# zhu-edward/DGSQP

Measured on NVIDIA B200. Metric: converged_game_solves_per_sec, higher is better.
Workload: dtype f64

## Files before the change

dgsqp_b200/csrc/cta.cuh:

```cuda
#pragma once
#include <math.h>
#include <stdint.h>

enum { PH_LIN_FULL = 0, PH_ADJ_FULL, PH_HESS, PH_PD_TRIDIAG, PH_PD_EIG, PH_CHOL, PH_TRINV, PH_GI, PH_LSQR,
       PH_LIN_GRAD, PH_ADJ_GRAD, PH_MERIT, PH_OTHER,
       PH_PD_SYM, PH_PD_EIGVAL, PH_PD_INVIT, PH_PD_BACK, PH_GI_SLACK, PH_GI_DZ, PH_GI_STEP, PH_GI_ADD, PH_GI_DROP, PH_QP_X0, PH_QP_WARM,
       PH_WS_D, PH_WS_QR, PH_WS_APPLY, PH_WS_MULT,
       DG_NPHASE };

#ifdef DG_HOSTSIM
#define DG_RSQRT(x) (1.0 / sqrt(x))
#define DG_ATOMIC_MIN(p, v) do { if ((v) < *(p)) *(p) = (v); } while (0)
#define DG_DEV static inline
#define DG_HD static inline
#define DG_DEVN static
#define DG_CONST static const
#define DG_RESTRICT
struct Cta {
  inline int tid() const { return 0; }
  inline int nt() const { return 1; }
  inline int lane() const { return 0; }
  inline int warp() const { return 0; }
  inline int nwarps() const { return 1; }
  static constexpr int wsz = 1;
  double* red = nullptr;
  inline void sync() {}
  inline double sum(double v) { return v; }
  inline double max(double v) { return v; }
  inline void max3(double& a, double& b, double& d) {}
  inline double min(double v) { return v; }
  inline int imin(int v) { return v; }
  inline int isum(int v) { return v; }
  inline void argmin(double v, int idx, double& ov, int& oi) { ov = v; oi = idx; }
  inline double warp_sum(double v) { return v; }
  template <int N> inline void warp_sum_n(double (&)[N]) {}
  inline void warp_argmin(double&, int&) {}
  inline void syncwarp() {}
  inline void sum2(double& a, double& b) {}
  inline void sum3(double& a, double& b, double& d) {}
  inline void sum4(double& a, double& b, double& d, double& e) {}
  inline int bcast0(int v) { return v; }
  inline void lap(int) {}
  inline void lapf(int) {}
  inline void lap2(int, int) {}
};
#else
#define DG_RSQRT(x) rsqrt(x)
#define DG_ATOMIC_MIN(p, v) atomicMin((p), (v))
#define DG_DEV __device__ __forceinline__
#define DG_HD __host__ __device__ __forceinline__
#define DG_DEVN __device__ __noinline__
#define DG_CONST __device__ const
#ifdef DG_NO_RESTRICT
#define DG_RESTRICT
#else
#define DG_RESTRICT __restrict__
#endif
__shared__ __align__(16) double dg_s_red[320];
__shared__ long long dg_s_ph[DG_NPHASE + 1];

struct Cta {
  __device__ __forceinline__ int tid() const { return (int)threadIdx.x; }
  __device__ __forceinline__ int nt() const { return (int)blockDim.x; }
  __device__ __forceinline__ int lane() const { return (int)(threadIdx.x & 31u); }
  __device__ __forceinline__ int warp() const { return (int)(threadIdx.x >> 5); }
  __device__ __forceinline__ int nwarps() const { return (int)((blockDim.x + 31u) >> 5); }
  static constexpr int wsz = 32;
  __device__ __forceinline__ void lap(int id) {
    if (tid() == 0) { long long t = clock64(); dg_s_ph[id] += t - dg_s_ph[DG_NPHASE]; dg_s_ph[DG_NPHASE] = t; }
  }
#ifdef DG_FINE_PHASES
  __device__ __forceinline__ void lapf(int id) { lap(id); }
  __device__ __forceinline__ void lap2(int, int fine) { lap(fine); }
#else
  __device__ __forceinline__ void lapf(int) {}
  __device__ __forceinline__ void lap2(int coarse, int) { lap(coarse); }
#endif
  __device__ __forceinline__ void sync() { __syncthreads(); }
  __device__ __forceinline__ double warp_sum(double v) {
#pragma unroll
    for (int o = 16; o > 0; o >>= 1) v += __shfl_xor_sync(0xffffffffu, v, o);
    return v;
  }
  template <int N>
  __device__ __forceinline__ void warp_sum_n(double (&v)[N]) {
#pragma unroll
    for (int o = 16; o > 0; o >>= 1) {
#pragma unroll
      for (int t = 0; t < N; ++t) v[t] += __shfl_xor_sync(0xffffffffu, v[t], o);
    }
  }
  __device__ __forceinline__ void warp_argmin(double& v, int& idx) {
#pragma unroll
    for (int o = 16; o > 0; o >>= 1) {
      const double v2 = __shfl_xor_sync(0xffffffffu, v, o);
      const int i2 = __shfl_xor_sync(0xffffffffu, idx, o);
      if (v2 < v || (v2 == v && i2 < idx)) { v = v2; idx = i2; }
    }
  }
  int flip = 0;
  __device__ __forceinline__ double* next_buf() { flip ^= 1; return dg_s_red + flip * 160; }
  __device__ __forceinline__ void syncwarp() { __syncwarp(); }
  __device__ __forceinline__ double tree16(const double* b) const {
    if (nwarps() == 8) {
      const double2 p0 = reinterpret_cast<const double2*>(b)[0], p1 = reinterpret_cast<const double2*>(b)[1];
      const double2 p2 = reinterpret_cast<const double2*>(b)[2], p3 = reinterpret_cast<const double2*>(b)[3];
      return ((p0.x + p0.y) + (p1.x + p1.y)) + ((p2.x + p2.y) + (p3.x + p3.y));
    }
    double t[16];
#pragma unroll
    for (int w = 0; w < 16; ++w) t[w] = w < nwarps() ? b[w] : 0.0;
#pragma unroll
    for (int s = 8; s > 0; s >>= 1)
#pragma unroll
      for (int w = 0; w < s; ++w) t[w] += t[w + s];
    return t[0];
  }
  __device__ __forceinline__ double sum(double v) {
    v = warp_sum(v);
    double* b = next_buf();
    if (lane() == 0) b[warp()] = v;
    __syncthreads();
    return tree16(b);
  }
  __device__ __forceinline__ void sum2(double& a0, double& a1) {
    a0 = warp_sum(a0); a1 = warp_sum(a1);
    double* b = next_buf();
    if (lane() == 0) { b[warp()] = a0; b[32 + warp()] = a1; }
    __syncthreads();
    a0 = tree16(b); a1 = tree16(b + 32);
  }
  __device__ __forceinline__ void sum3(double& a0, double& a1, double& a2) {
    a0 = warp_sum(a0); a1 = warp_sum(a1); a2 = warp_sum(a2);
    double* b = next_buf();
    if (lane() == 0) { b[warp()] = a0; b[32 + warp()] = a1; b[64 + warp()] = a2; }
    __syncthreads();
    a0 = tree16(b); a1 = tree16(b + 32); a2 = tree16(b + 64);
  }
  __device__ __forceinline__ void sum4(double& a0, double& a1, double& a2, double& a3) {
    a0 = warp_sum(a0); a1 = warp_sum(a1); a2 = warp_sum(a2); a3 = warp_sum(a3);
    double* b = next_buf();
    if (lane() == 0) { b[warp()] = a0; b[32 + warp()] = a1; b[64 + warp()] = a2; b[96 + warp()] = a3; }
    __syncthreads();
    a0 = tree16(b); a1 = tree16(b + 32); a2 = tree16(b + 64); a3 = tree16(b + 96);
  }
  __device__ __forceinline__ double max(double v) {
#pragma unroll
    for (int o = 16; o > 0; o >>= 1) v = fmax(v, __shfl_xor_sync(0xffffffffu, v, o));
    double* b = next_buf();
    if (lane() == 0) b[warp()] = v;
    __syncthreads();
    double r = b[0];
    for (int w = 1; w < nwarps(); ++w) r = fmax(r, b[w]);
    return r;
  }
  __device__ __forceinline__ void max3(double& a0, double& a1, double& a2) {
#pragma unroll
    for (int o = 16; o > 0; o >>= 1) {
      a0 = fmax(a0, __shfl_xor_sync(0xffffffffu, a0, o));
      a1 = fmax(a1, __shfl_xor_sync(0xffffffffu, a1, o));
      a2 = fmax(a2, __shfl_xor_sync(0xffffffffu, a2, o));
    }
    double* b = next_buf();
    if (lane() == 0) { b[warp()] = a0; b[32 + warp()] = a1; b[64 + warp()] = a2; }
    __syncthreads();
    double r0 = b[0], r1 = b[32], r2 = b[64];
    for (int w = 1; w < nwarps(); ++w) { r0 = fmax(r0, b[w]); r1 = fmax(r1, b[32 + w]); r2 = fmax(r2, b[64 + w]); }
    a0 = r0; a1 = r1; a2 = r2;
  }
  __device__ __forceinline__ double min(double v) { return -max(-v); }
  __device__ __forceinline__ int bcast0(int v) {
    int* b = (int*)next_buf();
    if (tid() == 0) b[0] = v;
    __syncthreads();
    return b[0];
  }
  __device__ __forceinline__ int imin(int v) {
#pragma unroll
    for (int o = 16; o > 0; o >>= 1) { int t = __shfl_xor_sync(0xffffffffu, v, o); v = t < v ? t : v; }
    int* b = (int*)next_buf();
    if (lane() == 0) b[warp()] = v;
    __syncthreads();
    int r = b[0];
    for (int w = 1; w < nwarps(); ++w) { int t = b[w]; r = t < r ? t : r; }
    return r;
  }
  __device__ __forceinline__ int isum(int v) {
#pragma unroll
    for (int o = 16; o > 0; o >>= 1) v += __shfl_xor_sync(0xffffffffu, v, o);
    int* b = (int*)next_buf();
    if (lane() == 0) b[warp()] = v;
    __syncthreads();
    int r = 0;
    for (int w = 0; w < nwarps(); ++w) r += b[w];
    return r;
  }
  __device__ __forceinline__ void argmin(double v, int idx, double& ov, int& oi) {
#pragma unroll
    for (int o = 16; o > 0; o >>= 1) {
      double v2 = __shfl_xor_sync(0xffffffffu, v, o);
      int i2 = __shfl_xor_sync(0xffffffffu, idx, o);
      if (v2 < v || (v2 == v && i2 < idx)) { v = v2; idx = i2; }
    }
    double* b = next_buf();
    if (lane() == 0) { b[warp()] = v; ((int*)(b + 32))[warp()] = idx; }
    __syncthreads();
    ov = b[0]; oi = ((int*)(b + 32))[0];
    for (int w = 1; w < nwarps(); ++w) {
      double v2 = b[w]; int i2 = ((int*)(b + 32))[w];
      if (v2 < ov || (v2 == ov && i2 < oi)) { ov = v2; oi = i2; }
    }
  }
};
#endif

#ifdef DG_HOSTSIM
#define DG_ASSUME_SHARED(p) do { } while (0)
#else
#define DG_ASSUME_SHARED(p) do { if (SM) __builtin_assume(__isShared((const void*)(p))); } while (0)
#endif

#ifdef DG_HOSTSIM
#include <chrono>
static inline double dg_now_ns() { return (double)std::chrono::duration_cast<std::chrono::nanoseconds>(std::chrono::steady_clock::now().time_since_epoch()).count(); }
#else
__device__ __forceinline__ double dg_now_ns() { unsigned long long t; asm volatile("mov.u64 %0, %%globaltimer;" : "=l"(t)); return (double)t; }
#endif

#define DG_FOR(i, n) for (int i = c.tid(); i < (n); i += c.nt())
#define DG_FOR_OFF(i, n, off) for (int i = (c.tid() + c.nt() - ((off) % c.nt())) % c.nt(); i < (n); i += c.nt())

struct Split2 { int i0, istep, g, G; };
DG_DEV Split2 split2(const Cta& c, int len) {
  int cw = (len + Cta::wsz - 1) / Cta::wsz * Cta::wsz;
  if (cw > c.nt()) cw = c.nt();
  if (cw < 1) cw = 1;
  Split2 s;
  s.G = c.nt() / cw; s.g = c.tid() / cw; s.i0 = c.tid() - s.g * cw; s.istep = cw;
  if (s.g >= s.G) s.i0 = len;
  return s;
}
```

dgsqp_b200/csrc/game_kkt.cuh:

```cuda
#pragma once

template <bool SM>
DG_DEVN void game_constraints(Cta& c, const GameDesc& G, const Dims& D_, const double* u, const double* up,
                              const double* x, double* g, const int* DG_RESTRICT rowtab) {
  const Dims D = D_;
  DG_ASSUME_SHARED(x); DG_ASSUME_SHARED(g); DG_ASSUME_SHARED(up);
  DG_FOR(r, D.m) {
    int k, kind, a, b;
    unpack_row(rowtab[r], k, kind, a, b);
    double val;
    if (kind == K_COLL) {
      double dx = x[k * D.nq + a * DG_NQA] - x[k * D.nq + b * DG_NQA];
      double dy = x[k * D.nq + a * DG_NQA + 1] - x[k * D.nq + b * DG_NQA + 1];
      double rr = G.obs_r[a] + G.obs_r[b];
      val = rr * rr - (dx * dx + dy * dy);
    } else if (kind == K_GAME) val = game_row_value(G, D, u, up, x, k, a, b);
    else if (kind == K_INUB) val = u[uidx(D, a, k, b)] - G.u_ub[b];
    else if (kind == K_INLB) val = G.u_lb[b] - u[uidx(D, a, k, b)];
    else if (kind == K_STUB) val = x[k * D.nq + a * DG_NQA + b] - game_state_ub(G);
    else val = game_state_lb(G) - x[k * D.nq + a * DG_NQA + b];
    g[r] = val;
  }
}

template <bool SM>
DG_DEVN void game_sens(Cta& c, const Dims& D_, const EvalBuf& E_) {
  const EvalBuf E = E_; DG_SH_EVAL(E); const Dims D = D_;
  const int twoN = D.twoN;
  DG_FOR(t, D.M * twoN) {
    int a = t / twoN, j = t - a * twoN, kj = j >> 1, cc = j & 1;
    double s[DG_NQA];
    const double* AB = E.AB + (kj * D.M + a) * DG_AB_SZ;
    for (int i = 0; i < DG_NQA; ++i) s[i] = AB[i * DG_AB_LD + DG_NQA + cc];
    for (int k = kj + 1; k <= D.N; ++k) {
      if (k > kj + 1) {
        const double* Ak = E.AB + ((k - 1) * D.M + a) * DG_AB_SZ;
        double ts[DG_NQA];
        for (int i = 0; i < DG_NQA; ++i) {
          double acc = 0.0;
          for (int jj = 0; jj < DG_NQA; ++jj) acc += Ak[i * DG_AB_LD + jj] * s[jj];
          ts[i] = acc;
        }
        for (int i = 0; i < DG_NQA; ++i) s[i] = ts[i];
      }
      double* Sk = E.S + sens_off(D, a, k, 0) + j;
      Sk[0] = s[0]; Sk[2 * k] = s[1]; Sk[4 * k] = s[DG_BOUND_STATE];
    }
  }
}

template <bool SM>
DG_DEV double sens_dot(const Dims& D, const EvalBuf& E, int a, int k, int row, const double* va) {
  const double* DG_RESTRICT Sk = E.S + sens_off(D, a, k, row);
  double a0 = 0.0, a1 = 0.0;
  for (int j = 0; j < 2 * k; j += 2) { a0 += Sk[j] * va[j]; a1 += Sk[j + 1] * va[j + 1]; }
  return a0 + a1;
}

template <bool SM>
DG_DEVN void game_G_times(Cta& c, const Dims& D_, const EvalBuf& E_, const double* v, double* y) {
  const EvalBuf E = E_; DG_SH_EVAL(E); const Dims D = D_;
  c.sync();
  DG_FOR(t, D.M * D.N * 3) {
    int a = t / (D.N * 3), rem = t - a * D.N * 3, k1 = rem / 3, row = rem - k1 * 3;
    E.tmpS[t] = sens_dot<SM>(D, E, a, k1 + 1, row, v + a * D.twoN);
  }
  c.sync();
  DG_FOR(r, D.m) {
    int k, kind, a, b;
    unpack_row(E.rowtab[r], k, kind, a, b);
    double val;
    if (kind == K_COLL) {
      double dx = E.x[k * D.nq + a * DG_NQA] - E.x[k * D.nq + b * DG_NQA];
      double dy = E.x[k * D.nq + a * DG_NQA + 1] - E.x[k * D.nq + b * DG_NQA + 1];
      const double* ta = E.tmpS + (a * D.N + (k - 1)) * 3;
      const double* tb = E.tmpS + (b * D.N + (k - 1)) * 3;
      val = -2.0 * (dx * (ta[0] - tb[0]) + dy * (ta[1] - tb[1]));
    } else if (kind == K_GAME) val = game_row_Gv(D, E, v, k, a, b);
    else if (kind == K_INUB) val = v[uidx(D, a, k, b)];
    else if (kind == K_INLB) val = -v[uidx(D, a, k, b)];
    else if (kind == K_STUB) val = E.tmpS[(a * D.N + (k - 1)) * 3 + 2];
    else val = -E.tmpS[(a * D.N + (k - 1)) * 3 + 2];
    y[r] = val;
  }
  c.sync();
}

template <bool SM>
DG_DEV void game_state_coefs(Cta& c, const Dims& D, const EvalBuf& E, const double* w, double* cf) {
  DG_FOR(t, D.M * D.N) {
    int a = t / D.N, k = t - a * D.N + 1;
    double cx = 0.0, cy = 0.0;
    for (int p = 0; p < D.P; ++p) {
      int i, j;
      pair_ij(D.M, p, i, j);
      if (i != a && j != a) continue;
      double dx = E.x[k * D.nq + i * DG_NQA] - E.x[k * D.nq + j * DG_NQA];
      double dy = E.x[k * D.nq + i * DG_NQA + 1] - E.x[k * D.nq + j * DG_NQA + 1];
      double wl = w[row_coll(D, k, p)] * (i == a ? -2.0 : 2.0);
      cx += wl * dx; cy += wl * dy;
    }
    game_row_coefs(D, E, w, k, a, cx, cy);
    cf[t * 3] = cx; cf[t * 3 + 1] = cy;
    cf[t * 3 + 2] = w[row_stub(D, k, a)] - w[row_stlb(D, k, a)];
  }
}

DG_DEV double game_GT_direct(const Dims& D, const double* w, int a, int k, int cc) {
  return game_row_GT_direct(D, w, a, k, cc, row_inub(D, k, a, cc), row_inlb(D, k, a, cc));
}

template <bool SM>
DG_DEVN void game_GT_times(Cta& c, const Dims& D_, const EvalBuf& E_, const double* w, double* y) {
  const EvalBuf E = E_; DG_SH_EVAL(E); const Dims D = D_;
  c.sync();
  game_state_coefs<SM>(c, D, E, w, E.cf);
  c.sync();
  DG_FOR(t, D.n) {
    int a = t / D.twoN, j = t - a * D.twoN, kj = j >> 1, cc = j & 1;
    double acc = game_GT_direct(D, w, a, kj, cc);
    for (int k = kj + 1; k <= D.N; ++k) {
      const double* Sk = E.S + sens_off(D, a, k, 0) + j;
      const double* cf = E.cf + (a * D.N + (k - 1)) * 3;
      acc += cf[0] * Sk[0] + cf[1] * Sk[2 * k] + cf[2] * Sk[4 * k];
    }
    y[t] = acc;
  }
  c.sync();
}

DG_DEV double game_G_entry(const Dims& D, const EvalBuf& E, const RowCoef& rc, int k, int kind, int a, int b, int t) {
  int ta = t / D.twoN, j = t - ta * D.twoN, kj = j >> 1, cc = j & 1;
  double val = 0.0;
  if (kind == K_COLL) {
    if ((ta == a || ta == b) && kj < k) {
      double dx = E.x[k * D.nq + a * DG_NQA] - E.x[k * D.nq + b * DG_NQA];
      double dy = E.x[k * D.nq + a * DG_NQA + 1] - E.x[k * D.nq + b * DG_NQA + 1];
      const double* Sk = E.S + sens_off(D, ta, k, 0) + j;
      double sg = ta == a ? -2.0 : 2.0;
      val = sg * (dx * Sk[0] + dy * Sk[2 * k]);
    }
  } else if (kind == K_GAME) game_row_G(D, E, rc, k, a, b, ta, j, kj, cc, val);
  else if (kind == K_INUB) { if (ta == a && kj == k && cc == b) val = 1.0; }
  else if (kind == K_INLB) { if (ta == a && kj == k && cc == b) val = -1.0; }
  else {
    if (ta == a && kj < k) {
      double sv = E.S[sens_off(D, ta, k, 2) + j];
      val = kind == K_STUB ? sv : -sv;
    }
  }
  return val;
}

DG_DEV bool game_G_sparse(const Dims& D, int r, int& t1, int& t2) {
  int k, kind, a, b;
  decode_row(D, r, k, kind, a, b);
  t1 = t2 = -1;
  if (kind == K_INUB) { t1 = uidx(D, a, k, b) << 1; return true; }
  if (kind == K_INLB) { t1 = (uidx(D, a, k, b) << 1) | 1; return true; }
  if (kind == K_GAME) return game_row_sparse(D, k, a, b, t1, t2);
  return false;
}

template <bool SM>
DG_DEVN void game_G_row(Cta& c, const Dims& D_, const EvalBuf& E_, int r, double* out) {
  const EvalBuf E = E_; DG_SH_EVAL(E); const Dims D = D_;
  int k, kind, a, b;
  decode_row(D, r, k, kind, a, b);
  RowCoef rc;
  game_row_prep(D, E, k, kind, a, b, rc);
  DG_FOR(t, D.n) out[t] = game_G_entry(D, E, rc, k, kind, a, b, t);
  c.sync();
}

template <bool SM>
DG_DEVN void game_G_cols(Cta& c, const Dims& D_, const EvalBuf& E_, const int* ids, int cnt, double* out, int ldo) {
  const EvalBuf E = E_; DG_SH_EVAL(E); const Dims D = D_;
  for (int col = c.warp(); col < cnt; col += c.nwarps()) {
    int k, kind, a, b;
    decode_row(D, ids[col], k, kind, a, b);
    RowCoef rc;
    game_row_prep(D, E, k, kind, a, b, rc);
    for (int t = c.lane(); t < D.n; t += c.wsz) out[t * ldo + col] = game_G_entry(D, E, rc, k, kind, a, b, t);
  }
}

DG_DEV double con_lx(const GameDesc& G, const Dims& D, const double* x, const double* l, int k, int idx) {
  int a = idx / DG_NQA, comp = idx - a * DG_NQA;
  if (comp == DG_BOUND_STATE) return l[row_stub(D, k, a)] - l[row_stlb(D, k, a)];
  if (comp > 1) return 0.0;
  double v = 0.0;
  for (int p = 0; p < D.P; ++p) {
    int i, j;
    pair_ij(D.M, p, i, j);
    if (i != a && j != a) continue;
    double dd = x[k * D.nq + i * DG_NQA + comp] - x[k * D.nq + j * DG_NQA + comp];
    v += l[row_coll(D, k, p)] * (i == a ? -2.0 : 2.0) * dd;
  }
  game_row_lx(G, D, x, l, k, a, comp, v);
  return v;
}

DG_DEV double con_lxx(const Dims& D, const double* l, int k, int i1, int i2) {
  int a1 = i1 / DG_NQA, c1 = i1 - a1 * DG_NQA, a2 = i2 / DG_NQA, c2 = i2 - a2 * DG_NQA;
  if (c1 > 1 || c1 != c2) return 0.0;
  double v = 0.0;
  for (int p = 0; p < D.P; ++p) {
    int i, j;
    pair_ij(D.M, p, i, j);
    double lp = l[row_coll(D, k, p)];
    if (a1 == a2) { if (a1 == i || a1 == j) v += -2.0 * lp; }
    else if ((a1 == i && a2 == j) || (a1 == j && a2 == i)) v += 2.0 * lp;
  }
  return v;
}

template <bool SM>
DG_DEVN void game_costates(Cta& c, const GameDesc& G, const Dims& D_, const EvalBuf& E_, const double* l) {
  const EvalBuf E = E_; DG_SH_EVAL(E); const Dims D = D_;
  DG_FOR(t, (D.M + 1) * D.M) {
    int f = t / D.M, b = t - f * D.M;
    double p[DG_NQA];
    double* out = E.cst + f * (D.N + 1) * D.nq;
    for (int i = 0; i < DG_NQA; ++i) {
      p[i] = f < D.M ? game_term_lx(G, D, E.x, f, b * DG_NQA + i) : con_lx(G, D, E.x, l, D.N, b * DG_NQA + i);
      out[D.N * D.nq + b * DG_NQA + i] = p[i];
    }
    for (int k = D.N - 1; k >= 0; --k) {
      const double* Ak = E.AB + (k * D.M + b) * DG_AB_SZ;
      double pn[DG_NQA];
      for (int j = 0; j < DG_NQA; ++j) {
        double acc = 0.0;
        if (k >= 1) acc = f < D.M ? game_stage_lx(G, D, E.x, f, k, b * DG_NQA + j) : con_lx(G, D, E.x, l, k, b * DG_NQA + j);
        for (int i = 0; i < DG_NQA; ++i) acc += Ak[i * DG_AB_LD + j] * p[i];
        pn[j] = acc;
      }
      for (int i = 0; i < DG_NQA; ++i) { p[i] = pn[i]; out[k * D.nq + b * DG_NQA + i] = pn[i]; }
    }
  }
}

template <bool SM>
DG_DEVN void game_gradients(Cta& c, const GameDesc& G, const Dims& D_, const EvalBuf& E_, const double* u,
                            const double* up, const double* l, double* qs) {
  const EvalBuf E = E_; DG_SH_EVAL(E); const Dims D = D_;
  DG_FOR(t, D.n) {
    int a = t / D.twoN, j = t - a * D.twoN, k = j >> 1, cc = j & 1;
    const double* Bk = E.AB + (k * D.M + a) * DG_AB_SZ;
    const double* pJ = E.cst + a * (D.N + 1) * D.nq + (k + 1) * D.nq + a * DG_NQA;
    const double* pC = E.cst + D.M * (D.N + 1) * D.nq + (k + 1) * D.nq + a * DG_NQA;
    double bj = 0.0, bc = 0.0;
    for (int i = 0; i < DG_NQA; ++i) { bj += Bk[i * DG_AB_LD + DG_NQA + cc] * pJ[i]; bc += Bk[i * DG_AB_LD + DG_NQA + cc] * pC[i]; }
    const InputGrad ig = game_input_grad(G, D, u, up, t, a, k, cc);
    E.q[t] = input_grad_plus(ig, bj);
    if (qs) {
      double bs = bj;
      for (int f = 0; f < D.M; ++f) {
        if (f == a) continue;
        const double* pF = E.cst + f * (D.N + 1) * D.nq + (k + 1) * D.nq + a * DG_NQA;
        for (int i = 0; i < DG_NQA; ++i) bs += Bk[i * DG_AB_LD + DG_NQA + cc] * pF[i];
      }
      qs[t] = input_grad_plus(ig, bs);
    }
    E.gtl[t] = game_GT_direct(D, l, a, k, cc) + bc;
  }
}

template <bool SM>
DG_DEVN void game_contract(Cta& c, const Dims& D_, const EvalBuf& E_) {
  const EvalBuf E = E_; DG_SH_EVAL(E); const Dims D = D_;
  DG_FOR(t, (D.M + 1) * D.N * D.M * DG_HC_SZ) {
    int e = t % DG_HC_SZ, r = t / DG_HC_SZ;
    int a = r % D.M; r /= D.M;
    int k = r % D.N, f = r / D.N;
    const double* p = E.cst + f * (D.N + 1) * D.nq + (k + 1) * D.nq + a * DG_NQA;
    const double* T = E.T2 + (k * D.M + a) * DG_T2_SZ;
    E.Hc[t] = game_contract_entry(p, T, e);
  }
}

template <bool SM>
DG_DEVN void game_hessian(Cta& c, const GameDesc& G, const Dims& D_, const EvalBuf& E_, const double* DG_RESTRICT l) {
  const EvalBuf E = E_; DG_SH_EVAL(E); const Dims D = D_;
  const int n = D.n, nq = D.nq, nu = D.nu, N = D.N, M = D.M, F = D.M + 1;
  double* Vcur = E.Vbuf;
  double* Vnext = E.Vbuf + F * nq * nq;
  double* DG_RESTRICT TV = E.Vbuf + 2 * F * nq * nq;
  DG_FOR(t, F * nq * nq) {
    int f = t / (nq * nq), e = t - f * nq * nq, i1 = e / nq, i2 = e - i1 * nq;
    Vcur[t] = f < M ? game_term_lxx(G, D, E.x, f, i1, i2) : con_lxx(D, l, N, i1, i2);
  }
  c.sync();
  double* DG_RESTRICT Qm = E.Q;
  for (int k = N - 1; k >= 0; --k) {
    const int nlater = n - (k + 1) * nu;
    const int nA1 = nlater * M, nA2 = F * nu * nq, nA3 = F * nq * nq;
    for (int t = c.tid(); t < nA1 + nA2 + nA3; t += c.nt()) {
      if (t < nA1) {
        const int b = t / nlater, r = (k + 1) * nu + (t - b * nlater);
        const int kr = r / nu, ar = (r - kr * nu) >> 1, cr = r & 1;
        const int rowQ = uidx(D, ar, kr, cr);
        double* DG_RESTRICT wr = E.Wrow + r;
        const double* DG_RESTRICT ABk = E.AB + (k * M + b) * DG_AB_SZ;
        double hM0 = 0.0, hM1 = 0.0, hA0 = 0.0, hA1 = 0.0, hB0 = 0.0, hB1 = 0.0;
        for (int f = 0; f < F; ++f) {
          double wv[DG_NQA];
#pragma unroll
          for (int i = 0; i < DG_NQA; ++i) wv[i] = wr[(f * nq + b * DG_NQA + i) * n];
          if (f == M || f == ar || f == b) {
            double v0 = 0.0, v1 = 0.0;
#pragma unroll
            for (int i = 0; i < DG_NQA; ++i) { v0 += wv[i] * ABk[i * DG_AB_LD + DG_NQA]; v1 += wv[i] * ABk[i * DG_AB_LD + DG_NQA + 1]; }
            if (f < M && kr == k + 1 && b == ar && f == ar) game_input_hess_prev(G, cr, v0, v1);
            if (f == M) { hM0 = v0; hM1 = v1; }
            if (f == ar) { hA0 = v0; hA1 = v1; }
            if (f == b) { hB0 = v0; hB1 = v1; }
          }
#pragma unroll
          for (int j = 0; j < DG_NQA; ++j) {
            double acc = 0.0;
#pragma unroll
            for (int i = 0; i < DG_NQA; ++i) acc += wv[i] * ABk[i * DG_AB_LD + j];
            wr[(f * nq + b * DG_NQA + j) * n] = acc;
          }
        }
        const int colQ = uidx(D, b, k, 0);
        Qm[rowQ * n + colQ] = hA0 + hM0;  Qm[rowQ * n + colQ + 1] = hA1 + hM1;
        Qm[colQ * n + rowQ] = hB0 + hM0;  Qm[(colQ + 1) * n + rowQ] = hB1 + hM1;
      } else if (t < nA1 + nA2) {
        const int e = t - nA1, f = e / (nu * nq), rem = e - f * nu * nq, rr = rem / nq, j = rem - rr * nq;
        const int ar = rr >> 1, cr = rr & 1;
        const double* DG_RESTRICT ABa = E.AB + (k * M + ar) * DG_AB_SZ;
        const double* DG_RESTRICT Vf = Vcur + f * nq * nq;
        double acc = 0.0;
#pragma unroll
        for (int i = 0; i < DG_NQA; ++i) acc += ABa[i * DG_AB_LD + DG_NQA + cr] * Vf[(ar * DG_NQA + i) * nq + j];
        TV[e] = acc;
      } else {
        const int tt = t - nA1 - nA2;
        const int f = tt / (nq * nq), e = tt - f * nq * nq;
        const int i1 = e / nq, i2 = e - i1 * nq, b1 = i1 / DG_NQA, b2 = i2 / DG_NQA, c1 = i1 - b1 * DG_NQA, c2 = i2 - b2 * DG_NQA;
        const double* DG_RESTRICT A1 = E.AB + (k * M + b1) * DG_AB_SZ;
        const double* DG_RESTRICT A2 = E.AB + (k * M + b2) * DG_AB_SZ;
        const double* DG_RESTRICT Vf = Vcur + f * nq * nq;
        double acc = f < M ? game_stage_lxx(G, D, f, k, i1, i2) : (k >= 1 ? con_lxx(D, l, k, i1, i2) : 0.0);
        if (b1 == b2) acc += hc_xx(E.Hc + ((f * N + k) * M + b1) * DG_HC_SZ, c1, c2);
#pragma unroll
        for (int i = 0; i < DG_NQA; ++i) {
          double rowacc = 0.0;
#pragma unroll
          for (int j = 0; j < DG_NQA; ++j) rowacc += Vf[(b1 * DG_NQA + i) * nq + b2 * DG_NQA + j] * A2[j * DG_AB_LD + c2];
          acc += A1[i * DG_AB_LD + c1] * rowacc;
        }
        Vnext[tt] = acc;
      }
    }
    c.sync();
    const int nB1 = F * nu * nq, nB2 = nu * M * 2;
    for (int t = c.tid(); t < nB1 + nB2; t += c.nt()) {
      if (t < nB1) {
        const int f = t / (nu * nq), rem = t - f * nu * nq, rr = rem / nq, q = rem - rr * nq, b = q / DG_NQA, j = q - b * DG_NQA;
        const int ar = rr >> 1, cr = rr & 1;
        const double* DG_RESTRICT ABb = E.AB + (k * M + b) * DG_AB_SZ;
        const double* DG_RESTRICT tv = TV + (f * nu + rr) * nq + b * DG_NQA;
        double acc = b == ar ? hc_ux(E.Hc + ((f * N + k) * M + ar) * DG_HC_SZ, cr, j) : 0.0;
#pragma unroll
        for (int i = 0; i < DG_NQA; ++i) acc += tv[i] * ABb[i * DG_AB_LD + j];
        E.Wrow[(f * nq + q) * n + k * nu + rr] = acc;
      } else {
        const int e = t - nB1, rr = e / (M * 2), rem = e - rr * M * 2, b = rem >> 1, cc = rem & 1;
        const int ar = rr >> 1, cr = rr & 1;
        const double* DG_RESTRICT ABb = E.AB + (k * M + b) * DG_AB_SZ;
        double vM = 0.0, vA = 0.0;
        const double* DG_RESTRICT tvM = TV + (M * nu + rr) * nq + b * DG_NQA;
        const double* DG_RESTRICT tvA = TV + (ar * nu + rr) * nq + b * DG_NQA;
#pragma unroll
        for (int i = 0; i < DG_NQA; ++i) { vM += tvM[i] * ABb[i * DG_AB_LD + DG_NQA + cc]; vA += tvA[i] * ABb[i * DG_AB_LD + DG_NQA + cc]; }
        if (b == ar) {
          vM += hc_uu(E.Hc + ((M * N + k) * M + ar) * DG_HC_SZ, cr, cc);
          vA += hc_uu(E.Hc + ((ar * N + k) * M + ar) * DG_HC_SZ, cr, cc);
          if (cc == cr) vA += game_input_hess(G, D, k, cc);
        }
        Qm[uidx(D, ar, k, cr) * n + uidx(D, b, k, cc)] = vA + vM;
      }
    }
    c.sync();
    double* tmp = Vcur; Vcur = Vnext; Vnext = tmp;
  }
}
```

Measured before the change: 2973.

## Parallelize costate backward recursion across warp lanes per state component

```diff
diff --git a/dgsqp_b200/csrc/cta.cuh b/dgsqp_b200/csrc/cta.cuh
--- a/dgsqp_b200/csrc/cta.cuh
+++ b/dgsqp_b200/csrc/cta.cuh
@@ -10,6 +10,7 @@
 
 #ifdef DG_HOSTSIM
 #define DG_RSQRT(x) (1.0 / sqrt(x))
+#define DG_FMA(a, b, c) ((a) * (b) + (c))
 #define DG_ATOMIC_MIN(p, v) do { if ((v) < *(p)) *(p) = (v); } while (0)
 #define DG_DEV static inline
 #define DG_HD static inline
@@ -46,6 +47,7 @@
 };
 #else
 #define DG_RSQRT(x) rsqrt(x)
+#define DG_FMA(a, b, c) __fma_rn((a), (b), (c))
 #define DG_ATOMIC_MIN(p, v) atomicMin((p), (v))
 #define DG_DEV __device__ __forceinline__
 #define DG_HD __host__ __device__ __forceinline__
diff --git a/dgsqp_b200/csrc/game_kkt.cuh b/dgsqp_b200/csrc/game_kkt.cuh
--- a/dgsqp_b200/csrc/game_kkt.cuh
+++ b/dgsqp_b200/csrc/game_kkt.cuh
@@ -28,7 +28,7 @@
   const EvalBuf E = E_; DG_SH_EVAL(E); const Dims D = D_;
   const int twoN = D.twoN;
   DG_FOR(t, D.M * twoN) {
-    int a = t / twoN, j = t - a * twoN, kj = j >> 1, cc = j & 1;
+    int j = t / D.M, a = t - j * D.M, kj = j >> 1, cc = j & 1;
     double s[DG_NQA];
     const double* AB = E.AB + (kj * D.M + a) * DG_AB_SZ;
     for (int i = 0; i < DG_NQA; ++i) s[i] = AB[i * DG_AB_LD + DG_NQA + cc];
@@ -218,25 +218,33 @@
 template <bool SM>
 DG_DEVN void game_costates(Cta& c, const GameDesc& G, const Dims& D_, const EvalBuf& E_, const double* l) {
   const EvalBuf E = E_; DG_SH_EVAL(E); const Dims D = D_;
-  DG_FOR(t, (D.M + 1) * D.M) {
-    int f = t / D.M, b = t - f * D.M;
-    double p[DG_NQA];
-    double* out = E.cst + f * (D.N + 1) * D.nq;
-    for (int i = 0; i < DG_NQA; ++i) {
-      p[i] = f < D.M ? game_term_lx(G, D, E.x, f, b * DG_NQA + i) : con_lx(G, D, E.x, l, D.N, b * DG_NQA + i);
-      out[D.N * D.nq + b * DG_NQA + i] = p[i];
-    }
-    for (int k = D.N - 1; k >= 0; --k) {
+  const int nch = (D.M + 1) * D.M;
+  const int cpw = c.wsz >= DG_NQA ? c.wsz / DG_NQA : nch;
+  const int ng = (nch + cpw - 1) / cpw, w = c.nwarps() - 1 - c.warp();
+  const int nown = ng > w ? (ng - w + c.nwarps() - 1) / c.nwarps() : 0;
+  const int per = cpw * DG_NQA;
+  for (int it = c.lane(); it < nown * per; it += c.wsz) {
+    const int o = it / per, e = it - o * per, t = (w + o * c.nwarps()) * cpw + e / DG_NQA, i = e % DG_NQA;
+    if (t >= nch) continue;
+    const int f = t / D.M, b = t - f * D.M;
+    E.cst[(f * (D.N + 1) + D.N) * D.nq + b * DG_NQA + i] =
+        f < D.M ? game_term_lx(G, D, E.x, f, b * DG_NQA + i) : con_lx(G, D, E.x, l, D.N, b * DG_NQA + i);
+  }
+  c.syncwarp();
+  for (int k = D.N - 1; k >= 0; --k) {
+    for (int it = c.lane(); it < nown * per; it += c.wsz) {
+      const int o = it / per, e = it - o * per, t = (w + o * c.nwarps()) * cpw + e / DG_NQA, j = e % DG_NQA;
+      if (t >= nch) continue;
+      const int f = t / D.M, b = t - f * D.M;
       const double* Ak = E.AB + (k * D.M + b) * DG_AB_SZ;
-      double pn[DG_NQA];
-      for (int j = 0; j < DG_NQA; ++j) {
-        double acc = 0.0;
-        if (k >= 1) acc = f < D.M ? game_stage_lx(G, D, E.x, f, k, b * DG_NQA + j) : con_lx(G, D, E.x, l, k, b * DG_NQA + j);
-        for (int i = 0; i < DG_NQA; ++i) acc += Ak[i * DG_AB_LD + j] * p[i];
-        pn[j] = acc;
-      }
-      for (int i = 0; i < DG_NQA; ++i) { p[i] = pn[i]; out[k * D.nq + b * DG_NQA + i] = pn[i]; }
-    }
+      double* out = E.cst + (f * (D.N + 1) + k) * D.nq + b * DG_NQA;
+      const double* p = out + D.nq;
+      double acc = 0.0;
+      if (k >= 1) acc = f < D.M ? game_stage_lx(G, D, E.x, f, k, b * DG_NQA + j) : con_lx(G, D, E.x, l, k, b * DG_NQA + j);
+      for (int i = 0; i < DG_NQA; ++i) acc = DG_FMA(Ak[i * DG_AB_LD + j], p[i], acc);
+      out[j] = acc;
+    }
+    c.syncwarp();
   }
 }
 
```

New measurement: 3138 (median of 6 runs). 5.5% higher.
